# twke18/SPML

Measured on AMD Instinct MI355X. Metric: images/sec (513x513) + k-means iters/sec, higher is better.
Workload: dtype f32

## Files before the change

### include/spml_hip.h

```cpp
#ifndef SPML_HIP_H_
#define SPML_HIP_H_

#include <stddef.h>
#include <stdint.h>

#ifdef __cplusplus
extern "C" {
#endif

typedef enum spml_status {
  SPML_OK = 0,
  SPML_ERR_INVALID_ARG = -1,
  SPML_ERR_UNSUPPORTED = -2,
  SPML_ERR_WORKSPACE = -3,
  SPML_ERR_LAUNCH = -4
} spml_status;

const char* spml_status_string(int status);

#define SPML_ABI_VERSION 8
int spml_abi_version(void);

int spml_set_deterministic(int on);
int spml_get_deterministic(void);
// ... 224 lines not shown


int spml_hl8_from_f32(const float* x, int64_t rows, int C, float* bound,
                      int compute_bound, void* out, void* stream);

int spml_hl8_weight_transposed_f32(const float* w, int Cout, int taps, int Cin,
                                   const float* bound, void* out, void* stream);

int spml_conv_hl8_supported(int K, int N, int taps);

int spml_conv_hl8_f32(const void* a, const float* a_bound, const void* b,
                      const float* b_bound, const float* addend,
                      const unsigned char* addend_mask, float* out,
                      int n_img, int H, int W, int K, int N, int taps, int dilation,
                      void* stream);

int spml_conv_hl8_stats_layout(int n_img, int H, int W, int K, int N, int taps,
                               int* chunks, int* chunk_rows);
int spml_conv_hl8_stats_f32(const void* a, const float* a_bound, const void* b,
                            const float* b_bound, float* out, float* chunk_stats,
                            float* zero_me, int n_img, int H, int W, int K, int N,
                            int taps, int dilation, void* stream);

int spml_conv_wgrad_hl8_supported(int K, int N, int taps);
size_t spml_conv_wgrad_workspace_bytes(int n_img, int H, int W, int K, int N, int taps);
int spml_conv_wgrad_hl8_f32(const void* dy, const float* dy_bound, const void* x,
                            const float* x_bound, float* dw, int n_img, int H, int W,
                            int K, int N, int taps, int dilation, void* ws,
                            size_t ws_bytes, void* stream);

int spml_conv_wgrad_pyramid_hl8_supported(int K, int N, int branches);
int spml_conv_tap_gather_f32(const float* z, const float* bias, float* out, int n_img, int H,
                             int W, int N, int branches, const int* dilations, void* stream);
size_t spml_conv_wgrad_pyramid_workspace_bytes(int n_img, int H, int W, int K, int N,
                                               int branches);
int spml_conv_wgrad_pyramid_hl8_f32(const void* dy, const float* dy_bound, const void* x,
                                    const float* x_bound, float* dw, int n_img, int H, int W,
                                    int K, int N, int branches, const int* dilations,
                                    void* ws, size_t ws_bytes, void* stream);

int spml_bn_stats_ext_f32(const float* x, int64_t R, int C, float* mean, float* m2,
                          float* cmax, float* cmin, void* ws, size_t ws_bytes,
                          void* stream);

int spml_bn_stats_ext_chunks_f32(const float* chunk_stats, int chunks, int chunk_rows,
                                 int64_t R, int C, float* mean, float* m2, float* cmax,
// ... 30 lines not shown

int spml_bn_fwd_hl8_f32(const float* x, const float* residual, const float* residual_bound,
                        int64_t R, int C, const float* gamma, const float* beta,
                        float* running_mean, float* running_var, float momentum, float eps,
                        int relu, float* y, void* y_hl8, float* y_bound,
                        unsigned char* relu_mask, float* mean, float* invstd, float* cmax,
                        float* cmin, void* ws, size_t ws_bytes, void* stream);

int spml_bn_fwd_hl8_chunks_f32(const float* x, const float* chunk_stats, int chunks,
                               int chunk_rows, const float* residual,
                               const float* residual_bound, int64_t R, int C,
                               const float* gamma, const float* beta, float* running_mean,
                               float* running_var, float momentum, float eps, int relu,
                               float* y, void* y_hl8, float* y_bound,
                               unsigned char* relu_mask, float* mean, float* invstd,
                               float* cmax, float* cmin, void* stream);

int spml_bn_bwd_hl8_f32(const float* dy, const float* y, const unsigned char* relu_mask,
                        const float* x, int64_t R, int C, const float* mean,
                        const float* invstd, const float* gamma, const float* cmax,
                        const float* cmin, float* d_gamma, float* d_beta, float* dx,
                        void* dx_hl8, float* dx_bound, float* d_residual, void* ws,
                        size_t ws_bytes, void* stream);

int spml_conv_hl8_pyramid_f32(const void* a, const float* a_bound, const void* b,
                              const float* b_bound, const float* bias, const float* addend,
                              float* out,
                              int n_img, int H, int W, int K, int N, int groups,
                              const int* dilations, void* stream);
int spml_hl8_weight_transposed_into_f32(const float* w, int Cout, int taps, int Cin,
                                        const float* bound, void* out, int taps_total,
                                        int tap_offset, void* stream);
int spml_absmax_bound_f32(const float* x, int64_t n, float* bound, int zero_first,
                          void* stream);

int spml_hl8_weight_set_f32(const float* const* w, const int* cout, const int* cin,
                            const int* taps, int n, float* bounds, void* const* fwd,
                            void* const* transposed, void* stream);

int spml_bn_finalize_ranks_f32(const float* stats, int world, int C, float eps,
                               float momentum, float* running_mean, float* running_var,
                               float* mean, float* invstd, float* total_count, void* stream);

int spml_conv_hl8_affine_f32(const void* a, const float* a_bound, const void* b,
                             const float* b_bound, const float* bias, const float* addend,
                             int relu, float* out, float* out_bound, int n_img, int H,
// ... 76 lines not shown
```

### spml_amd/_ffi.py

```python
import ctypes
import os
import threading
from ctypes import c_char_p, c_double, c_float, c_int, c_int64, c_size_t, c_void_p

import torch

_HERE = os.path.dirname(os.path.abspath(__file__))
LIB_PATH = os.environ.get('SPML_HIP_LIB') or os.path.join(_HERE, 'lib', 'libspml_hip.so')

_lib = None
_lock = threading.Lock()

_P = c_void_p
_SIGNATURES = {
    'spml_status_string': (c_char_p, [c_int]),
    'spml_abi_version': (c_int, []),
    'spml_normalize_concat_loc_f32': (c_int, [_P, c_int, c_int, c_int, c_int, _P, _P, _P, _P, _P]),
    'spml_normalize_concat_loc_bwd_f32': (c_int, [_P, c_int, c_int, c_int, c_int, _P, _P, _P, _P, _P, _P]),
    'spml_normalize_concat_local_f32': (c_int, [_P, c_int, c_int, c_int, c_int, _P, c_int, _P, _P, _P, _P]),
    'spml_normalize_concat_local_nhwc_supported': (c_int, [c_int, c_int]),
    'spml_normalize_concat_local_nhwc_f32': (c_int, [_P, c_int, c_int, c_int, c_int, _P, c_int, _P, _P, _P, _P]),
    'spml_normalize_concat_local_nhwc_bwd_f32': (c_int, [_P, c_int, c_int, c_int, c_int, _P, c_int, _P, _P, _P,
                                                         _P, _P]),
    'spml_normalize_concat_local_bwd_f32': (c_int, [_P, c_int, c_int, c_int, c_int, _P, c_int, _P, _P, _P,
# ... 32 lines not shown
    'spml_segsort_nll_batched_workspace_bytes': (c_size_t, [c_int, _P, _P, c_int]),
    'spml_segsort_nll_batched_fwd_f32': (c_int, [_P, _P, _P, _P, _P, _P, _P, c_int, c_int, c_float, c_int,
                                                 _P, _P, _P, c_size_t, _P]),
    'spml_segsort_nll_batched_bwd_f32': (c_int, [_P, _P, _P, _P, _P, _P, _P, c_int, c_int, c_float, c_int,
                                                 _P, _P, _P, _P, _P, c_size_t, _P]),
    'spml_topk_workspace_bytes': (c_size_t, [c_int64, c_int64, c_int, c_int]),
    'spml_topk_affinity_f32': (c_int, [_P, c_int64, _P, c_int64, c_int, c_int, _P, _P, _P, c_float,
                                       _P, _P, _P, c_size_t, _P]),
    'spml_affinity_workspace_bytes': (c_size_t, [c_int, c_int, c_int64]),
    'spml_affinity_transition_f32': (c_int, [_P, c_int, c_int, c_int64, c_float, c_int, _P, _P, c_size_t,
                                             _P]),
    'spml_bn_workspace_bytes': (c_size_t, [c_int64, c_int]),
    'spml_bn_act_fwd_f32': (c_int, [_P, _P, c_int64, c_int, _P, _P, _P, _P, c_float, c_float, c_int, _P, _P, _P,
                                    _P, c_size_t, _P]),
    'spml_bn_act_bwd_f32': (c_int, [_P, _P, _P, c_int64, c_int, _P, _P, _P, _P, _P, _P, _P, _P, c_size_t, _P]),
    'spml_hl8_from_f32': (c_int, [_P, c_int64, c_int, _P, c_int, _P, _P]),
    'spml_hl8_weight_transposed_f32': (c_int, [_P, c_int, c_int, c_int, _P, _P, _P]),
    'spml_conv_hl8_supported': (c_int, [c_int, c_int, c_int]),
    'spml_conv_hl8_f32': (c_int, [_P, _P, _P, _P, _P, _P, _P, c_int, c_int, c_int, c_int, c_int, c_int, c_int, _P]),
    'spml_conv_hl8_stats_layout': (c_int, [c_int, c_int, c_int, c_int, c_int, c_int, _P, _P]),
    'spml_conv_hl8_stats_f32': (c_int, [_P, _P, _P, _P, _P, _P, _P, c_int, c_int, c_int, c_int, c_int, c_int, c_int, _P]),
    'spml_bn_fwd_hl8_chunks_f32': (c_int, [_P, _P, c_int, c_int, _P, _P, c_int64, c_int, _P, _P, _P, _P, c_float, c_float,
                                           c_int, _P, _P, _P, _P, _P, _P, _P, _P, _P]),
    'spml_conv_wgrad_hl8_supported': (c_int, [c_int, c_int, c_int]),
    'spml_conv_wgrad_workspace_bytes': (c_size_t, [c_int, c_int, c_int, c_int, c_int, c_int]),
    'spml_conv_wgrad_hl8_f32': (c_int, [_P, _P, _P, _P, _P, c_int, c_int, c_int, c_int, c_int, c_int, c_int, _P,
                                        c_size_t, _P]),
    'spml_conv_wgrad_pyramid_hl8_supported': (c_int, [c_int, c_int, c_int]),
    'spml_conv_tap_gather_f32': (c_int, [_P, _P, _P, c_int, c_int, c_int, c_int, c_int, _P, _P]),
    'spml_conv_wgrad_pyramid_workspace_bytes': (c_size_t, [c_int, c_int, c_int, c_int, c_int, c_int]),
    'spml_conv_wgrad_pyramid_hl8_f32': (c_int, [_P, _P, _P, _P, _P, c_int, c_int, c_int, c_int, c_int, c_int, _P, _P,
                                                c_size_t, _P]),
    'spml_bn_stats_ext_f32': (c_int, [_P, c_int64, c_int, _P, _P, _P, _P, _P, c_size_t, _P]),
    'spml_bn_stats_ext_chunks_f32': (c_int, [_P, c_int, c_int, c_int64, c_int, _P, _P, _P, _P, _P]),
    'spml_bn_finalize_f32': (c_int, [_P, _P, c_int, c_double, c_float, c_float, _P, _P, _P, _P]),
    'spml_bn_act_apply_hl8_f32': (c_int, [_P, _P, _P, c_int64, c_int, _P, _P, _P, _P, _P, _P, c_int, _P, _P, _P, _P,
                                          _P]),
    'spml_bn_act_bwd_reduce_ext_f32': (c_int, [_P, _P, _P, _P, c_int64, c_int, _P, _P, _P, _P, _P, _P, c_size_t, _P]),
    'spml_bn_act_bwd_apply_hl8_f32': (c_int, [_P, _P, _P, _P, c_int64, c_int, _P, _P, _P, _P, _P, _P, _P, _P,
                                              c_double, _P, _P, _P, _P, _P, _P]),
    'spml_bn_fwd_hl8_f32': (c_int, [_P, _P, _P, c_int64, c_int, _P, _P, _P, _P, c_float, c_float, c_int, _P, _P, _P, _P,
                                    _P, _P, _P, _P, _P, c_size_t, _P]),
    'spml_bn_bwd_hl8_f32': (c_int, [_P, _P, _P, _P, c_int64, c_int, _P, _P, _P, _P, _P, _P, _P, _P, _P, _P, _P, _P,
                                    c_size_t, _P]),
    'spml_conv_hl8_pyramid_f32': (c_int, [_P, _P, _P, _P, _P, _P, _P, c_int, c_int, c_int, c_int, c_int, c_int, _P,
                                          _P]),
# ... 849 lines not shown
  def __init__(self, data, chunks, chunk_rows, bound):
    self.data, self.chunks, self.chunk_rows, self.bound = data, chunks, chunk_rows, bound


def conv_hl8_stats(a, b, n_img, h, w, taps, dilation=1):
  import ctypes
  k, n = a.channels, b.rows
  chunks, rows = ctypes.c_int(0), ctypes.c_int(0)
  if os.environ.get('SPML_CONV_BN_STATS') == '0' or lib().spml_conv_hl8_stats_layout(
      n_img, h, w, k, n, taps, ctypes.byref(chunks), ctypes.byref(rows)) != 0:
    return conv_hl8(a, b, n_img, h, w, taps, dilation), None
  if a.rows != n_img * h * w or b.channels != taps * k:
    raise SpmlHipError('conv_hl8_stats: operand shapes do not match')
  dev = a.data.device
  out = torch.empty((n_img, n, h, w), dtype=torch.float32, device=dev, memory_format=torch.channels_last)
  st = torch.empty((4, chunks.value, n), dtype=torch.float32, device=dev)
  bound = _f32(1, dev)
  check(lib().spml_conv_hl8_stats_f32(ptr(a.data), c_void_p(a.bound.data_ptr()), ptr(b.data),
                                      c_void_p(b.bound.data_ptr()), _ptr_any(out), _dp(st), _dp(bound), n_img, h, w,
                                      k, n, taps, dilation, stream_ptr()), 'spml_conv_hl8_stats_f32')
  return out, ChunkStats(st, chunks.value, rows.value, bound)


def conv_wgrad_hl8_supported(k, n, taps):
  return bool(lib().spml_conv_wgrad_hl8_supported(int(k), int(n), int(taps)))


_wgrad_ws = {}


def conv_wgrad_hl8(dy, x, n_img, h, w, taps, dilation=1):
  n, k = dy.channels, x.channels
  if dy.rows != n_img * h * w or x.rows != dy.rows:
    raise SpmlHipError('conv_wgrad_hl8: operand shapes do not match')
  need = lib().spml_conv_wgrad_workspace_bytes(n_img, h, w, k, n, taps)
  key = (dy.data.device.index, torch.cuda.current_stream().cuda_stream)
  ws = _wgrad_ws.get(key)
  if ws is None or ws.numel() < need:
    ws = workspace(need, dy.data.device)
    _wgrad_ws[key] = ws
  side = 3 if taps == 9 else 1
  dw = torch.empty((n, k, side, side), dtype=torch.float32, device=dy.data.device,
                   memory_format=torch.channels_last)
  check(lib().spml_conv_wgrad_hl8_f32(ptr(dy.data), c_void_p(dy.bound.data_ptr()), ptr(x.data),
                                      c_void_p(x.bound.data_ptr()), _ptr_any(dw), n_img, h, w, k, n, taps,
                                      dilation, ptr(ws), ws.numel(), stream_ptr()), 'spml_conv_wgrad_hl8_f32')
# ... 65 lines not shown


def bn_finalize(mean, m2, count, eps, momentum, running_mean, running_var):
  invstd = torch.empty_like(mean)
  check(lib().spml_bn_finalize_f32(_dp(mean), _dp(m2), mean.numel(), float(count), float(eps), float(momentum),
                                   _dp(running_mean), _dp(running_var), _dp(invstd), stream_ptr()),
        'spml_bn_finalize_f32')
  return invstd


def bn_act_apply_hl8(x, rows, channels, residual, residual_bound, mean, invstd, gamma, beta, cmax, cmin, relu,
                     want_f32, want_hl8, like=None, want_mask=False):
  y = torch.empty_like(x if like is None else like) if want_f32 else None
  yh = torch.empty((rows * channels * 4,), dtype=torch.uint8, device=x.device) if want_hl8 else None
  bound = _f32(1, x.device)
  mask = torch.empty((rows * (channels // 4),), dtype=torch.uint8, device=x.device) if want_mask else None
  check(lib().spml_bn_act_apply_hl8_f32(
      _ptr_any(x), _ptr_any(residual, True), _dp(residual_bound), rows, channels, _dp(mean), _dp(invstd),
      ptr(gamma, torch.float32), ptr(beta, torch.float32), _dp(cmax), _dp(cmin), int(bool(relu)), _ptr_any(y, True),
      _dp(yh), _dp(bound), _dp(mask), stream_ptr()), 'spml_bn_act_apply_hl8_f32')
  return y, (Hl8(yh, bound, rows, channels) if want_hl8 else None), bound, mask


def bn_act_bwd_reduce_ext(dy, y, relu_mask, x, rows, channels, mean, invstd):
  st = torch.empty((3, channels), dtype=torch.float32, device=dy.device)
  ws = _bn_workspace(rows, channels, dy.device)
  check(lib().spml_bn_act_bwd_reduce_ext_f32(
      _ptr_any(dy), _ptr_any(y, True), _dp(relu_mask), _ptr_any(x), rows, channels,
      _dp(mean), _dp(invstd), _dp(st[0]), _dp(st[1]), _dp(st[2]), ptr(ws), ws.numel(), stream_ptr()),
        'spml_bn_act_bwd_reduce_ext_f32')
  return st


def bn_act_bwd_apply_hl8(dy, y, relu_mask, x, rows, channels, mean, invstd, gamma, s0, s1, max_dz, cmax, cmin, count,
                         want_dx_f32=False, want_dx_hl8=True, want_dres=False):
  dx = torch.empty_like(dy) if want_dx_f32 else None
  dxh = torch.empty((rows * channels * 4,), dtype=torch.uint8, device=dy.device) if want_dx_hl8 else None
  bound = _f32(1, dy.device) if want_dx_hl8 else None
  dres = torch.empty_like(dy) if want_dres else None
  count, count_dev = _count_args(count)
  check(lib().spml_bn_act_bwd_apply_hl8_f32(
      _ptr_any(dy), _ptr_any(y, True), _dp(relu_mask), _ptr_any(x), rows, channels,
      _dp(mean), _dp(invstd), ptr(gamma, torch.float32), _dp(s0), _dp(s1), _dp(max_dz), _dp(cmax), _dp(cmin),
      count, count_dev, _ptr_any(dx, True), _dp(dxh), _dp(bound), _ptr_any(dres, True), stream_ptr()),
        'spml_bn_act_bwd_apply_hl8_f32')
  return dx, (Hl8(dxh, bound, rows, channels) if want_dx_hl8 else None), dres


def bn_fwd_hl8(x, rows, channels, residual, residual_bound, gamma, beta, running_mean, running_var, momentum, eps,
               relu, want_f32, want_hl8, want_mask, chunk_stats=None):
  y = torch.empty_like(x) if want_f32 else None
  yh = torch.empty((rows * channels * 4,), dtype=torch.uint8, device=x.device) if want_hl8 else None
  bound = _f32(1, x.device) if chunk_stats is None else chunk_stats.bound
  mask = torch.empty((rows * (channels // 4),), dtype=torch.uint8, device=x.device) if want_mask else None
  st = torch.empty((4, channels), dtype=torch.float32, device=x.device)
  if chunk_stats is not None:
    check(lib().spml_bn_fwd_hl8_chunks_f32(
        _ptr_any(x), _dp(chunk_stats.data), chunk_stats.chunks, chunk_stats.chunk_rows, _ptr_any(residual, True),
        _dp(residual_bound), rows, channels, ptr(gamma, torch.float32), ptr(beta, torch.float32), _dp(running_mean),
        _dp(running_var), float(momentum), float(eps), int(bool(relu)), _ptr_any(y, True), _dp(yh), _dp(bound),
        _dp(mask), _dp(st[0]), _dp(st[1]), _dp(st[2]), _dp(st[3]), stream_ptr()), 'spml_bn_fwd_hl8_chunks_f32')
    return y, (Hl8(yh, bound, rows, channels) if want_hl8 else None), bound, mask, (st[0], st[1], st[2], st[3])
  ws = _bn_workspace(rows, channels, x.device)
  check(lib().spml_bn_fwd_hl8_f32(
      _ptr_any(x), _ptr_any(residual, True), _dp(residual_bound), rows, channels, ptr(gamma, torch.float32),
      ptr(beta, torch.float32), _dp(running_mean), _dp(running_var), float(momentum), float(eps), int(bool(relu)),
      _ptr_any(y, True), _dp(yh), _dp(bound), _dp(mask), _dp(st[0]), _dp(st[1]), _dp(st[2]), _dp(st[3]), ptr(ws),
      ws.numel(), stream_ptr()), 'spml_bn_fwd_hl8_f32')
  return y, (Hl8(yh, bound, rows, channels) if want_hl8 else None), bound, mask, (st[0], st[1], st[2], st[3])


def bn_bwd_hl8(dy, relu_mask, x, rows, channels, saved, gamma, want_dres=False):
  mean, invstd, cmax, cmin = saved
  dxh = torch.empty((rows * channels * 4,), dtype=torch.uint8, device=dy.device)
  bound = _f32(1, dy.device)
  dres = torch.empty_like(dy) if want_dres else None
  dgb = torch.empty((2, channels), dtype=torch.float32, device=dy.device)
  ws = _bn_workspace(rows, channels, dy.device)
  check(lib().spml_bn_bwd_hl8_f32(
      _ptr_any(dy), c_void_p(0), _dp(relu_mask), _ptr_any(x), rows, channels, _dp(mean), _dp(invstd),
      ptr(gamma, torch.float32), _dp(cmax), _dp(cmin), _dp(dgb[0]), _dp(dgb[1]), c_void_p(0), _dp(dxh), _dp(bound),
      _ptr_any(dres, True), ptr(ws), ws.numel(), stream_ptr()), 'spml_bn_bwd_hl8_f32')
  return Hl8(dxh, bound, rows, channels), dres, dgb[0], dgb[1]


def conv_hl8_pyramid_dgrad(dy, weights, dilations, n_img, h, w):
  groups = len(weights)
  cout, cin = weights[0].shape[0], weights[0].shape[1]
  dev = dy.data.device
  bound = torch.empty((1,), dtype=torch.float32, device=dev)
  wl = [wt.detach().contiguous(memory_format=torch.channels_last) for wt in weights]
  for g, wt in enumerate(wl):
    check(lib().spml_absmax_bound_f32(_ptr_any(wt), wt.numel(), _dp(bound), int(g == 0), stream_ptr()),
          'spml_absmax_bound_f32')
  b = torch.empty((cin * 9 * groups * cout * 4,), dtype=torch.uint8, device=dev)
  for g, wt in enumerate(wl):
    check(lib().spml_hl8_weight_transposed_into_f32(_ptr_any(wt), cout, 9, cin, _dp(bound), ptr(b), 9 * groups, 9 * g,
                                                    stream_ptr()), 'spml_hl8_weight_transposed_into_f32')
  out = torch.empty((n_img, cin, h, w), dtype=torch.float32, device=dev, memory_format=torch.channels_last)
# ... 161 lines not shown
```

### spml_amd/csrc/bn_act.hip

```cpp
#include "common.hpp"

namespace spml {
namespace {


__device__ __forceinline__ float4v relu_mask_bits(float4v dz, const unsigned char* __restrict__ mask, size_t row,
                                                  int C, int q) {
  const unsigned m = mask[row * (size_t)(C >> 2) + q];
#pragma unroll
  for (int e = 0; e < 4; ++e) dz[e] = (m >> e) & 1u ? dz[e] : 0.f;
  return dz;
}

__device__ __forceinline__ float bn_pow2_scale(float bound) {
  if (!(bound > 0.f) || bound > 1e38f) return 1.f;
  int e;
  (void)frexpf(bound, &e);
  e = 14 - e;
  e = e < -100 ? -100 : (e > 100 ? 100 : e);
  return ldexpf(1.f, e);
}

__device__ __forceinline__ void store_hl8_quad(uint2* __restrict__ out, size_t row, int C, int q, float4v v,
                                               float s) {
// ... 790 lines not shown
    return SPML_ERR_UNSUPPORTED;
  if (!ws || ws_bytes < spml_bn_workspace_bytes(R, C)) return SPML_ERR_WORKSPACE;
  const int chunks = bn_chunks(R, C), cq = bn_cq(C), crows = bn_chunk_rows(R, C), arows = bn_apply_rows(R, C);
  float* pa = static_cast<float*>(ws);
  float* pb = pa + (size_t)chunks * C;
  float* pc = pb + (size_t)chunks * C;
  float* max_dz = pc + (size_t)chunks * C;
  hipStream_t s = (hipStream_t)stream;
  const int mask = y ? 1 : (relu_mask ? 2 : 0);
  SPML_BN_PARTIAL1(mask, dim3(((C >> 2) + cq - 1) / cq, chunks), dim3(256), 0, s, x, dy, y, mean, R, C, cq, crows, pa, pb,
                   relu_mask, pc, (float*)nullptr, dx_hl8 ? dx_bound : (float*)nullptr);
  hipLaunchKernelGGL(bn_merge<1>, dim3((C + kMergeCh - 1) / kMergeCh), dim3(kMergeCh * kMergeLanes), 0, s, pa, pb, R,
                     C, chunks, crows, invstd, d_beta, d_gamma, BnFinal{0, 0.f, 0.f, nullptr, nullptr},
                     (const float*)pc, (const float*)nullptr, max_dz, (float*)nullptr,
                     BnBound{dx_hl8 ? dx_bound : nullptr, nullptr, gamma, nullptr, mean, cmax, cmin, (float)(1.0 / (double)R)});
  if (!dx && !dx_hl8 && !d_residual) return launch_status();
  const dim3 grid(((C >> 2) + cq - 1) / cq, (unsigned)((R + arows - 1) / arows));
  SPML_BN_BY_MASK(bn_bwd_apply, mask, grid, dim3(256), 0, s, dy, y, x, R, C, cq, arows, mean, invstd, gamma,
                  (const float*)d_beta, (const float*)d_gamma, (float)(1.0 / (double)R), (const float*)nullptr, dx,
                  d_residual, relu_mask, static_cast<uint2*>(dx_hl8), (const float*)dx_bound);
  return launch_status();
}

extern "C" int spml_bn_finalize_ranks_f32(const float* stats, int world, int C, float eps, float momentum,
                                          float* running_mean, float* running_var, float* mean, float* invstd,
                                          float* total_count, void* stream) {
  if (!stats || !mean || !invstd || world < 1 || C <= 0) return SPML_ERR_INVALID_ARG;
  hipLaunchKernelGGL(bn_finalize_ranks, dim3((C + 255) / 256), dim3(256), 0, (hipStream_t)stream, C, world, stats, eps,
                     momentum, running_mean, running_var, mean, invstd, total_count);
  return launch_status();
}
```

### spml_amd/csrc/conv.hip

```cpp
#include "common.hpp"

#include <math.h>
#include <stdlib.h>

#ifndef SPML_CONV_EXP
#define SPML_CONV_EXP 0
#endif

namespace spml {
namespace {

typedef const __attribute__((address_space(1))) void* gptr_t;
typedef __attribute__((address_space(3))) void* lptr_t;

__device__ uint4 g_zero_page[16];

__device__ __forceinline__ float pow2_scale(float bound) {
  if (!(bound > 0.f) || bound > 1e38f) return 1.f;
  int e;
  (void)frexpf(bound, &e);
  e = 14 - e;
  e = e < -100 ? -100 : (e > 100 ? 100 : e);
  return ldexpf(1.f, e);
}

__device__ __forceinline__ void split_unscaled(const float (&v)[8], float s, half8& h, half8& l) {
#pragma unroll
  for (int j = 0; j < 8; ++j) {
    const float x = v[j] * s;
    const _Float16 hj = (_Float16)x;
    h[j] = hj;
    l[j] = (_Float16)(x - (float)hj);
  }
// ... 111 lines not shown
      th[(2 * tu + 1) * 8 + (co & 7)] = ll.e[e];
    }
  }
}

struct ConvArgs {
  const uint4* a;
  const uint4* b;
  const float* a_bound;
  const float* b_bound;
  const float* addend;
  const unsigned char* addend_mask;
  const float* bias;
  int relu;
  float* out_bound;
  float* out;
  int64_t R;
  int H, W, K, N, taps, dil;
  int n_col_tiles, n_tiles;
  int dils[4];
  int tap_groups;
  float* stats;
  float* stats_zero;
};

template <int RB, int kStages, int WGS, int RG, bool CHUNK = false, int NC = 4>
__global__ __launch_bounds__(64 * NC * RG, WGS) void conv_gemm(const ConvArgs a) {
  constexpr int kABlocks = 2 * RB * RG;
  constexpr int kBlocks = kABlocks + 4 * NC;
  constexpr int kStage = kBlocks * 1024;
  constexpr int kWaves = NC * RG;
  constexpr int NQ = (kABlocks + kWaves - 1) / kWaves;
  extern __shared__ __attribute__((aligned(1024))) unsigned char lds[];
  const int lane = threadIdx.x & 63, wave = threadIdx.x >> 6;
  const int wc = wave % NC, wg = wave / NC;
  const int lr = lane & 31;
  const int drow = lane >> 2, dpiece = ((lane & 3) - (drow >> 2)) & 3;
  const unsigned foff_h = (unsigned)((lr >> 4) * 1024 + 16 * (4 * (lr & 15) + (((lane >> 5) * 2 + ((lr & 15) >> 2)) & 3)));
  const unsigned foff_l = (unsigned)((lr >> 4) * 1024 + 16 * (4 * (lr & 15) + (((lane >> 5) * 2 + 1 + ((lr & 15) >> 2)) & 3)));

  unsigned long long exp_c0 = 0, exp_r0 = 0;
  if (SPML_CONV_EXP & 16) { exp_c0 = __builtin_amdgcn_s_memtime(); exp_r0 = __builtin_amdgcn_s_memrealtime(); }
  int t = blockIdx.x;
  if ((a.n_tiles & 7) == 0) t = (t & 7) * (a.n_tiles >> 3) + (t >> 3);
  const int row_tile = t / a.n_col_tiles, col_tile = t - row_tile * a.n_col_tiles;
  const int64_t m0 = (int64_t)row_tile * (RG * RB * 32);
  const int n0 = col_tile * (64 * NC) + wc * 64;
  const int k8 = a.K >> 3, nk = a.K >> 4;
  const int hw = a.H * a.W;
  const int tpg = a.taps / (int)gridDim.y, tap_begin = (int)blockIdx.y * tpg, tap_end = tap_begin + tpg;
// ... 142 lines not shown
      acc[i][1] = mfma32(ah[c], bh1, acc[i][1]);
      } else {
        asm volatile("" :: "v"(al[c]), "v"(ah[c]), "v"(bh0), "v"(bl0), "v"(bh1), "v"(bl1));
      }
    }
    if (CHUNK && (s & 63) == 63) {
#pragma unroll
      for (int i = 0; i < RB; ++i)
#pragma unroll
        for (int j = 0; j < 2; ++j)
#pragma unroll
          for (int r = 0; r < 16; ++r) { tot[i][j][r] += acc[i][j][r]; acc[i][j][r] = 0.f; }
    }
  }
  if (CHUNK) {
#pragma unroll
    for (int i = 0; i < RB; ++i)
#pragma unroll
      for (int j = 0; j < 2; ++j)
#pragma unroll
        for (int r = 0; r < 16; ++r) acc[i][j][r] += tot[i][j][r];
  }

  const float mult = 1.0f / ((a.a_bound ? pow2_scale(*a.a_bound) : 1.f) * (a.b_bound ? pow2_scale(*a.b_bound) : 1.f));
  float vmax = 0.f;
#pragma unroll
  for (int i = 0; i < RB; ++i)
#pragma unroll
    for (int r = 0; r < 16; ++r) {
      const int64_t row = m0 + (wg * RB + i) * 32 + acc_row(r, lane);
      if (row < a.R) {
#pragma unroll
        for (int j = 0; j < 2; ++j) {
          const size_t o = (size_t)row * a.N + n0 + j * 32 + lr;
          float v = acc[i][j][r] * mult;
          if (gridDim.y > 1) {
            if (a.bias && blockIdx.y == 0) v += a.bias[n0 + j * 32 + lr];
            unsafeAtomicAdd(a.out + o, v);
            continue;
          }
          if (a.bias) v += a.bias[n0 + j * 32 + lr];
          if (a.addend) {
            float ad = a.addend[o];
            if (a.addend_mask) ad = (a.addend_mask[o >> 2] >> (o & 3)) & 1 ? ad : 0.f;
            v += ad;
          }
// ... 41 lines not shown
          dst[0] = mean;
          dst[plane] = m2;
          dst[2 * plane] = hi;
          dst[3 * plane] = lo;
        }
      }
    }
  }
  if ((SPML_CONV_EXP & 32) && blockIdx.x == 7 && lane == 0) {
#pragma unroll
    for (int i = 0; i < 4; ++i) a.out[8 + wave * 4 + i] = (float)exp_ph[i];
  }
  if ((SPML_CONV_EXP & 16) && blockIdx.x == 7 && threadIdx.x == 0) {
    a.out[0] = (float)(__builtin_amdgcn_s_memtime() - exp_c0);
    a.out[1] = (float)(__builtin_amdgcn_s_memrealtime() - exp_r0);
  }
  if (a.out_bound) {
#pragma unroll
    for (int o = 32; o > 0; o >>= 1) vmax = fmaxf(vmax, __shfl_xor(vmax, o, kWave));
    if (lane == 0) atomicMax(reinterpret_cast<unsigned*>(a.out_bound), __float_as_uint(vmax));
  }
}

template <int RB, int kStages, int WGS, int RG = 1, bool CHUNK = false, int NC = 4>
int launch_conv(const ConvArgs& a0, hipStream_t s) {
  ConvArgs a = a0;
  a.n_col_tiles = a.N / (64 * NC);
  const int64_t row_tiles = (a.R + RG * RB * 32 - 1) / (RG * RB * 32);
  a.n_tiles = (int)(row_tiles * a.n_col_tiles);
  auto kern = conv_gemm<RB, kStages, WGS, RG, CHUNK, NC>;
  const int lds = kStages * (2 * RB * RG + 4 * NC) * 1024;
  (void)hipFuncSetAttribute(reinterpret_cast<const void*>(kern), hipFuncAttributeMaxDynamicSharedMemorySize, lds);
  const int groups = a.tap_groups > 1 ? a.tap_groups : 1;
  if (groups > 1 && hipMemsetAsync(a.out, 0, (size_t)a.R * a.N * sizeof(float), s) != hipSuccess) return SPML_ERR_LAUNCH;
  hipLaunchKernelGGL(kern, dim3(a.n_tiles, groups), dim3(64 * NC * RG), lds, s, a);
  return launch_status();
}

template <bool CHUNK>
int launch_conv_narrow(const ConvArgs& c, hipStream_t s) {
  if ((c.N & 127) == 0) return launch_conv<CHUNK ? 3 : 4, 3, 2, 2, CHUNK, 2>(c, s);
  const char* e = getenv("SPML_CONV_NARROW_RB");
  if (e && e[0] == '3') return launch_conv<3, 3, 1, 4, CHUNK, 1>(c, s);
  return launch_conv<2, 3, 2, 4, CHUNK, 1>(c, s);
}

inline bool chunk_long_reduction(int64_t k_total) {
  int64_t min_k = 4096;
  if (const char* e = getenv("SPML_CONV_CHUNK_MIN_K")) min_k = atoll(e);
  return k_total >= min_k;
}

inline int pick_rb(int64_t R, int N) {
// ... 392 lines not shown
                                       float* out, float* chunk_stats, float* zero_me, int n_img, int H, int W,
                                       int K, int N, int taps, int dilation, void* stream) {
  if (!a || !b || !out || !chunk_stats || n_img <= 0 || H <= 0 || W <= 0 || dilation < 1) return SPML_ERR_INVALID_ARG;
  int chunks = 0, rows = 0;
  if (spml_conv_hl8_stats_layout(n_img, H, W, K, N, taps, &chunks, &rows) != SPML_OK || !al16(a) || !al16(b) ||
      !al16(out))
    return SPML_ERR_UNSUPPORTED;
  ConvArgs c{};
  c.a = static_cast<const uint4*>(a);
  c.b = static_cast<const uint4*>(b);
  c.a_bound = a_bound;
  c.b_bound = b_bound;
  c.out = out;
  c.stats = chunk_stats;
  c.stats_zero = zero_me;
  c.R = (int64_t)n_img * H * W;
  c.H = H; c.W = W; c.K = K; c.N = N; c.taps = taps; c.dil = dilation;
  hipStream_t s = (hipStream_t)stream;
  if (chunk_long_reduction((int64_t)c.K * c.taps)) return launch_conv<3, 3, 2, 1, true>(c, s);
  switch (rows / 32) {
    case 3: return launch_conv<3, 3, 2>(c, s);
    case 5: return launch_conv<5, 3, 2>(c, s);
    default: return launch_conv<4, 3, 2>(c, s);
  }
}

extern "C" int spml_conv_hl8_affine_f32(const void* a, const float* a_bound, const void* b, const float* b_bound,
                                        const float* bias, const float* addend, int relu, float* out,
                                        float* out_bound, int n_img, int H, int W, int K, int N, int taps,
                                        int dilation, void* stream) {
  if (!a || !b || !out || n_img <= 0 || H <= 0 || W <= 0 || dilation < 1) return SPML_ERR_INVALID_ARG;
  if (!spml_conv_hl8_supported(K, N, taps) || !al16(a) || !al16(b) || !al16(out) || (addend && !al16(addend)))
    return SPML_ERR_UNSUPPORTED;
  ConvArgs c{};
  c.a = static_cast<const uint4*>(a);
  c.b = static_cast<const uint4*>(b);
  c.a_bound = a_bound;
  c.b_bound = b_bound;
  c.bias = bias;
  c.addend = addend;
  c.relu = relu;
  c.out = out;
  c.out_bound = out_bound;
  c.R = (int64_t)n_img * H * W;
  c.H = H; c.W = W; c.K = K; c.N = N; c.taps = taps; c.dil = dilation;
  hipStream_t s = (hipStream_t)stream;
// ... 216 lines not shown
```

### spml_amd/mc_bottleneck.py

```python
import os

import torch
import torch.distributed as dist

from spml_amd import _ffi
from spml_amd._cache import BoundedCache


def _group_of(bn):
  if isinstance(bn, torch.nn.SyncBatchNorm) and dist.is_available() and dist.is_initialized():
    return bn.process_group if bn.process_group is not None else dist.group.WORLD
  return None


def available(block, x, allow_forward_only=True):
  if os.environ.get('SPML_NO_MC_CONV') == '1' or not (x.is_cuda and x.dtype == torch.float32 and x.dim() == 4):
    return False
  if not block.training or block.stride != 1 or not x.is_contiguous(memory_format=torch.channels_last):
    return False
  convs = [block.conv1, block.conv2, block.conv3] + ([block.downsample[0]] if block.downsample is not None else [])
  if os.environ.get('SPML_MC_NARROW_UNITS') == '0' and any(
      (c.in_channels & 255) or (c.out_channels & 255) for c in convs):
    return False
  bns = [block.bn1, block.bn2, block.bn3] + ([block.downsample[1]] if block.downsample is not None else [])
# ... 93 lines not shown
      return
    if gathered is None:
      st = _ffi.bn_stats_ext(a, rows, channels, chunk_stats=chunk_stats)
      allst = torch.empty((world * 3, channels), dtype=st.dtype, device=st.device)
      dist.all_gather_into_tensor(allst, st[:3], group=group)
      allst = allst.view(world, 3, channels)
    else:
      allst, st = gathered
    if bn.num_batches_tracked is not None:
      if counters is not None:
        counters.append(bn.num_batches_tracked)
      else:
        bn.num_batches_tracked.add_(1)
    mean, invstd, self.count = _ffi.bn_finalize_ranks(allst, bn.eps, bn.momentum, bn.running_mean, bn.running_var)
    _touch(bn)
    cmax, cmin = st[3], st[4]
    self.y, self.yh, self.bound, self.mask = _ffi.bn_act_apply_hl8(
        a, rows, channels, residual, residual_bound, mean, invstd, bn.weight, bn.bias, cmax, cmin, relu,
        want_f32, want_hl8, want_mask=relu)
    self.saved = (mean, invstd, cmax, cmin)


def _bn_backward(dy, a, rows, channels, gamma, saved, count, group, world, mask, want_dres=False,
                 want_dx_f32=False):
  if world == 1:
    dxh, dres, d_gamma, d_beta = _ffi.bn_bwd_hl8(dy, mask, a, rows, channels, saved, gamma, want_dres=want_dres)
    return None, dxh, dres, d_gamma, d_beta
  mean, invstd, cmax, cmin = saved
  st = _ffi.bn_act_bwd_reduce_ext(dy, None, mask, a, rows, channels, mean, invstd)
  local = st[:2].clone()
  d_beta, d_gamma = local[0], local[1]
  dist.all_reduce(st[:2], group=group)
  dx, dxh, dres = _ffi.bn_act_bwd_apply_hl8(dy, None, mask, a, rows, channels, mean, invstd, gamma, st[0], st[1],
                                            st[2], cmax, cmin, count, want_dx_f32=want_dx_f32, want_dx_hl8=True,
                                            want_dres=want_dres)
  return dx, dxh, dres, d_gamma, d_beta


def sync_pair(bn_a, a_a, chunk_a, bn_b, a_b, chunk_b, rows, channels):
  group = _group_of(bn_a)
  if group is None or _group_of(bn_b) is not group or dist.get_world_size(group) == 1:
    return None, None
  world = dist.get_world_size(group)
  st_a = _ffi.bn_stats_ext(a_a, rows, channels, chunk_stats=chunk_a)
  st_b = _ffi.bn_stats_ext(a_b, rows, channels, chunk_stats=chunk_b)
  loc = torch.cat([st_a[:3], st_b[:3]], dim=1)
  allst = torch.empty((world * 3, 2 * channels), dtype=loc.dtype, device=loc.device)
  dist.all_gather_into_tensor(allst, loc, group=group)
  allst = allst.view(world, 3, 2 * channels)
  return (allst[:, :, :channels].contiguous(), st_a), (allst[:, :, channels:].contiguous(), st_b)


# ... 90 lines not shown
    rows = n * h * w
    (xh_d, xh_b, a1, y1_d, y1_b, a2, y2_d, y2_b, a3, m3, m1, m2, w1t_d, w1t_b, w2t_d, w2t_b, w3t_d, w3t_b, g1, g2,
     g3) = t[:21]
    s1, s2, s3 = t[21:25], t[25:29], t[29:33]
    has_ds = len(t) > 33
    H = _ffi.Hl8
    xh, y1h, y2h = H(xh_d, xh_b, rows, cin), H(y1_d, y1_b, rows, width), H(y2_d, y2_b, rows, width)
    w1t, w2t, w3t = H(w1t_d, w1t_b, cin, width), H(w2t_d, w2t_b, width, 9 * width), H(w3t_d, w3t_b, width, cout)
    if not d_out.is_contiguous(memory_format=torch.channels_last):
      d_out = d_out.contiguous(memory_format=torch.channels_last)
    need_x = ctx.needs_input_grad[1]
    m = ctx.bn_meta
    dwd = dgd = dbd = dad = None
    pair = has_ds and m[2][2] > 1 and m[3][1] is m[2][1]
    if pair:
      da3, dad, dg3, db3, dgd, dbd = _bn_backward_pair(d_out, m3, a3, g3, s3, t[33], t[36], t[37:41], rows, cout,
                                                       m[2][0], m[2][1])
      dres = None
    else:
      _, da3, dres, dg3, db3 = _bn_backward(d_out, a3, rows, cout, g3, s3, m[2][0], m[2][1], m[2][2], m3,
                                            want_dres=has_ds)
    side = _side_stream(d_out.device)
    dw3 = _wgrad(side, da3, y2h, n, h, w, 1)
    dy2 = _ffi.conv_hl8(da3, w3t, n, h, w, 1)
    del da3
    _, da2, _, dg2, db2 = _bn_backward(dy2, a2, rows, width, g2, s2, m[1][0], m[1][1], m[1][2], m2)
    dw2 = _wgrad(side, da2, y1h, n, h, w, 9, dil)
    dy1 = _ffi.conv_hl8(da2, w2t, n, h, w, 9, dil)
    del da2, dy2
    _, da1, _, dg1, db1 = _bn_backward(dy1, a1, rows, width, g1, s1, m[0][0], m[0][1], m[0][2], m1)
    dw1 = _wgrad(side, da1, xh, n, h, w, 1)
    dx = None
    if has_ds:
      ad, wdt_d, wdt_b, gd = t[33:37]
      sd = t[37:41]
      if not pair:
        _, dad, _, dgd, dbd = _bn_backward(dres, ad, rows, cout, gd, sd, m[3][0], m[3][1], m[3][2], None)
      dwd = _wgrad(side, dad, xh, n, h, w, 1)
      if need_x:
        dx = _ffi.conv_hl8(da1, w1t, n, h, w, 1)
        dx = _ffi.conv_hl8(dad, H(wdt_d, wdt_b, cin, cout), n, h, w, 1, addend=dx)
    elif need_x:
      dx = _ffi.conv_hl8(da1, w1t, n, h, w, 1, addend=d_out, addend_mask=m3)
    if side is not None:
      torch.cuda.current_stream().wait_stream(side)
    return (None, dx, None, None, dw1, dg1, db1, dw2, dg2, db2, dw3, dg3, db3, dwd, dgd, dbd)


class _ConvBnAct(torch.autograd.Function):

  @staticmethod
  def forward(ctx, conv, bn, x, weight, gamma, beta):
    n, cin, h, w = x.shape
# ... 61 lines not shown
```

Before: 136.3.

## Fuse BN-backward reduction statistics into dgrad conv epilogue in bottleneck backward

Adds a BSTAT variant of the conv GEMM epilogue that, while storing the conv output, loads the BN input and ReLU mask and accumulates per-chunk sum(dz), sum(dz*(x-mean)) and max|dz|. BN backward then merges these chunk stats instead of making a separate reduction pass over dy and x. This is meant to remove one full read of the activation gradient and the saved input per BN layer in the bottleneck backward. In exchange the conv epilogue does extra loads, which raises register pressure and can lower conv occupancy.

```diff
diff --git a/include/spml_hip.h b/include/spml_hip.h
--- a/include/spml_hip.h
+++ b/include/spml_hip.h
@@ -270,6 +270,14 @@
                             float* zero_me, int n_img, int H, int W, int K, int N,
                             int taps, int dilation, void* stream);
 
+int spml_conv_hl8_bwd_stats_layout(int n_img, int H, int W, int K, int N, int taps,
+                                   int* chunks, int* chunk_rows);
+int spml_conv_hl8_bwd_stats_f32(const void* a, const float* a_bound, const void* b,
+                                const float* b_bound, float* out, const float* bn_x,
+                                const unsigned char* relu_mask, const float* bn_mean,
+                                float* chunk_stats, float* zero_me, int n_img, int H, int W,
+                                int K, int N, int taps, int dilation, void* stream);
+
 int spml_conv_wgrad_hl8_supported(int K, int N, int taps);
 size_t spml_conv_wgrad_workspace_bytes(int n_img, int H, int W, int K, int N, int taps);
 int spml_conv_wgrad_hl8_f32(const void* dy, const float* dy_bound, const void* x,
@@ -346,6 +354,17 @@
                         const float* cmin, float* d_gamma, float* d_beta, float* dx,
                         void* dx_hl8, float* dx_bound, float* d_residual, void* ws,
                         size_t ws_bytes, void* stream);
+
+int spml_bn_bwd_hl8_chunks_f32(const float* dy, const unsigned char* relu_mask, const float* x,
+                               const float* chunk_stats, int chunks, int chunk_rows, int64_t R,
+                               int C, const float* mean, const float* invstd, const float* gamma,
+                               const float* cmax, const float* cmin, float* d_gamma,
+                               float* d_beta, float* max_dz, float* dx, void* dx_hl8,
+                               float* dx_bound, float* d_residual, void* stream);
+
+int spml_bn_act_bwd_reduce_ext_chunks_f32(const float* chunk_stats, int chunks, int chunk_rows,
+                                          int64_t R, int C, const float* invstd, float* sum_dz,
+                                          float* sum_dz_xhat, float* max_dz, void* stream);
 
 int spml_conv_hl8_pyramid_f32(const void* a, const float* a_bound, const void* b,
                               const float* b_bound, const float* bias, const float* addend,
diff --git a/spml_amd/_ffi.py b/spml_amd/_ffi.py
--- a/spml_amd/_ffi.py
+++ b/spml_amd/_ffi.py
@@ -78,6 +78,12 @@
     'spml_conv_hl8_stats_f32': (c_int, [_P, _P, _P, _P, _P, _P, _P, c_int, c_int, c_int, c_int, c_int, c_int, c_int, _P]),
     'spml_bn_fwd_hl8_chunks_f32': (c_int, [_P, _P, c_int, c_int, _P, _P, c_int64, c_int, _P, _P, _P, _P, c_float, c_float,
                                            c_int, _P, _P, _P, _P, _P, _P, _P, _P, _P]),
+    'spml_conv_hl8_bwd_stats_layout': (c_int, [c_int, c_int, c_int, c_int, c_int, c_int, _P, _P]),
+    'spml_conv_hl8_bwd_stats_f32': (c_int, [_P, _P, _P, _P, _P, _P, _P, _P, _P, _P, c_int, c_int, c_int, c_int, c_int,
+                                            c_int, c_int, _P]),
+    'spml_bn_bwd_hl8_chunks_f32': (c_int, [_P, _P, _P, _P, c_int, c_int, c_int64, c_int, _P, _P, _P, _P, _P, _P, _P, _P,
+                                           _P, _P, _P, _P, _P]),
+    'spml_bn_act_bwd_reduce_ext_chunks_f32': (c_int, [_P, c_int, c_int, c_int64, c_int, _P, _P, _P, _P, _P]),
     'spml_conv_wgrad_hl8_supported': (c_int, [c_int, c_int, c_int]),
     'spml_conv_wgrad_workspace_bytes': (c_size_t, [c_int, c_int, c_int, c_int, c_int, c_int]),
     'spml_conv_wgrad_hl8_f32': (c_int, [_P, _P, _P, _P, _P, c_int, c_int, c_int, c_int, c_int, c_int, c_int, _P,
@@ -973,6 +979,27 @@
   return out, ChunkStats(st, chunks.value, rows.value, bound)
 
 
+def conv_hl8_bwd_stats(a, b, n_img, h, w, taps, dilation, bn_x, relu_mask, bn_mean):
+  import ctypes
+  k, n = a.channels, b.rows
+  chunks, rows = ctypes.c_int(0), ctypes.c_int(0)
+  if relu_mask is None or os.environ.get('SPML_CONV_BN_BWD_STATS') == '0' or lib().spml_conv_hl8_bwd_stats_layout(
+      n_img, h, w, k, n, taps, ctypes.byref(chunks), ctypes.byref(rows)) != 0:
+    return conv_hl8(a, b, n_img, h, w, taps, dilation), None
+  if a.rows != n_img * h * w or b.channels != taps * k or bn_x.numel() != a.rows * n or \
+      relu_mask.numel() != a.rows * (n // 4) or bn_mean.numel() != n:
+    raise SpmlHipError('conv_hl8_bwd_stats: operand shapes do not match')
+  dev = a.data.device
+  out = torch.empty((n_img, n, h, w), dtype=torch.float32, device=dev, memory_format=torch.channels_last)
+  st = torch.empty((3, chunks.value, n), dtype=torch.float32, device=dev)
+  bound = _f32(1, dev)
+  check(lib().spml_conv_hl8_bwd_stats_f32(ptr(a.data), c_void_p(a.bound.data_ptr()), ptr(b.data),
+                                          c_void_p(b.bound.data_ptr()), _ptr_any(out), _ptr_any(bn_x), _dp(relu_mask),
+                                          _dp(bn_mean), _dp(st), _dp(bound), n_img, h, w, k, n, taps, dilation,
+                                          stream_ptr()), 'spml_conv_hl8_bwd_stats_f32')
+  return out, ChunkStats(st, chunks.value, rows.value, bound)
+
+
 def conv_wgrad_hl8_supported(k, n, taps):
   return bool(lib().spml_conv_wgrad_hl8_supported(int(k), int(n), int(taps)))
 
@@ -1084,8 +1111,13 @@
   return y, (Hl8(yh, bound, rows, channels) if want_hl8 else None), bound, mask
 
 
-def bn_act_bwd_reduce_ext(dy, y, relu_mask, x, rows, channels, mean, invstd):
+def bn_act_bwd_reduce_ext(dy, y, relu_mask, x, rows, channels, mean, invstd, chunk_stats=None):
   st = torch.empty((3, channels), dtype=torch.float32, device=dy.device)
+  if chunk_stats is not None:
+    check(lib().spml_bn_act_bwd_reduce_ext_chunks_f32(
+        _dp(chunk_stats.data), chunk_stats.chunks, chunk_stats.chunk_rows, rows, channels, _dp(invstd), _dp(st[0]),
+        _dp(st[1]), _dp(st[2]), stream_ptr()), 'spml_bn_act_bwd_reduce_ext_chunks_f32')
+    return st
   ws = _bn_workspace(rows, channels, dy.device)
   check(lib().spml_bn_act_bwd_reduce_ext_f32(
       _ptr_any(dy), _ptr_any(y, True), _dp(relu_mask), _ptr_any(x), rows, channels,
@@ -1132,11 +1164,20 @@
   return y, (Hl8(yh, bound, rows, channels) if want_hl8 else None), bound, mask, (st[0], st[1], st[2], st[3])
 
 
-def bn_bwd_hl8(dy, relu_mask, x, rows, channels, saved, gamma, want_dres=False):
+def bn_bwd_hl8(dy, relu_mask, x, rows, channels, saved, gamma, want_dres=False, chunk_stats=None):
   mean, invstd, cmax, cmin = saved
   dxh = torch.empty((rows * channels * 4,), dtype=torch.uint8, device=dy.device)
+  dres = torch.empty_like(dy) if want_dres else None
+  if chunk_stats is not None:
+    bound = chunk_stats.bound
+    dgb = torch.empty((3, channels), dtype=torch.float32, device=dy.device)
+    check(lib().spml_bn_bwd_hl8_chunks_f32(
+        _ptr_any(dy), _dp(relu_mask), _ptr_any(x), _dp(chunk_stats.data), chunk_stats.chunks, chunk_stats.chunk_rows,
+        rows, channels, _dp(mean), _dp(invstd), ptr(gamma, torch.float32), _dp(cmax), _dp(cmin), _dp(dgb[0]),
+        _dp(dgb[1]), _dp(dgb[2]), c_void_p(0), _dp(dxh), _dp(bound), _ptr_any(dres, True), stream_ptr()),
+          'spml_bn_bwd_hl8_chunks_f32')
+    return Hl8(dxh, bound, rows, channels), dres, dgb[0], dgb[1]
   bound = _f32(1, dy.device)
-  dres = torch.empty_like(dy) if want_dres else None
   dgb = torch.empty((2, channels), dtype=torch.float32, device=dy.device)
   ws = _bn_workspace(rows, channels, dy.device)
   check(lib().spml_bn_bwd_hl8_f32(
diff --git a/spml_amd/csrc/bn_act.hip b/spml_amd/csrc/bn_act.hip
--- a/spml_amd/csrc/bn_act.hip
+++ b/spml_amd/csrc/bn_act.hip
@@ -836,6 +836,53 @@
   return launch_status();
 }
 
+extern "C" int spml_bn_bwd_hl8_chunks_f32(const float* dy, const unsigned char* relu_mask, const float* x,
+                                          const float* chunk_stats, int chunks, int chunk_rows, int64_t R, int C,
+                                          const float* mean, const float* invstd, const float* gamma,
+                                          const float* cmax, const float* cmin, float* d_gamma, float* d_beta,
+                                          float* max_dz, float* dx, void* dx_hl8, float* dx_bound, float* d_residual,
+                                          void* stream) {
+  if (!dy || !x || !chunk_stats || !mean || !invstd || !gamma || !cmax || !cmin || !d_gamma || !d_beta || !max_dz ||
+      R <= 0 || C <= 0 || chunks <= 0 || chunk_rows <= 0 || (int64_t)chunks * chunk_rows < R ||
+      (int64_t)(chunks - 1) * chunk_rows >= R || (dx_hl8 && !dx_bound))
+    return SPML_ERR_INVALID_ARG;
+  if ((C & 7) || !bn_ok(dy) || !bn_ok(x) || (dx && !bn_ok(dx)) || (dx_hl8 && !bn_ok(dx_hl8)) ||
+      (d_residual && !bn_ok(d_residual)) || !bn_ok(mean))
+    return SPML_ERR_UNSUPPORTED;
+  const int cq = bn_cq(C), arows = bn_apply_rows(R, C);
+  const float* pa = chunk_stats;
+  const float* pb = pa + (size_t)chunks * C;
+  const float* pc = pb + (size_t)chunks * C;
+  hipStream_t s = (hipStream_t)stream;
+  const int mask = relu_mask ? 2 : 0;
+  hipLaunchKernelGGL(bn_merge<1>, dim3((C + kMergeCh - 1) / kMergeCh), dim3(kMergeCh * kMergeLanes), 0, s, pa, pb, R,
+                     C, chunks, chunk_rows, invstd, d_beta, d_gamma, BnFinal{0, 0.f, 0.f, nullptr, nullptr}, pc,
+                     (const float*)nullptr, max_dz, (float*)nullptr,
+                     BnBound{dx_hl8 ? dx_bound : nullptr, nullptr, gamma, nullptr, mean, cmax, cmin, (float)(1.0 / (double)R)});
+  if (!dx && !dx_hl8 && !d_residual) return launch_status();
+  const dim3 grid(((C >> 2) + cq - 1) / cq, (unsigned)((R + arows - 1) / arows));
+  SPML_BN_BY_MASK(bn_bwd_apply, mask, grid, dim3(256), 0, s, dy, (const float*)nullptr, x, R, C, cq, arows, mean, invstd,
+                  gamma, (const float*)d_beta, (const float*)d_gamma, (float)(1.0 / (double)R), (const float*)nullptr, dx,
+                  d_residual, relu_mask, static_cast<uint2*>(dx_hl8), (const float*)dx_bound);
+  return launch_status();
+}
+
+extern "C" int spml_bn_act_bwd_reduce_ext_chunks_f32(const float* chunk_stats, int chunks, int chunk_rows, int64_t R,
+                                                     int C, const float* invstd, float* sum_dz, float* sum_dz_xhat,
+                                                     float* max_dz, void* stream) {
+  if (!chunk_stats || !invstd || !sum_dz || !sum_dz_xhat || !max_dz || R <= 0 || C <= 0 || chunks <= 0 ||
+      chunk_rows <= 0 || (int64_t)chunks * chunk_rows < R || (int64_t)(chunks - 1) * chunk_rows >= R)
+    return SPML_ERR_INVALID_ARG;
+  const float* pa = chunk_stats;
+  const float* pb = pa + (size_t)chunks * C;
+  const float* pc = pb + (size_t)chunks * C;
+  hipLaunchKernelGGL(bn_merge<1>, dim3((C + kMergeCh - 1) / kMergeCh), dim3(kMergeCh * kMergeLanes), 0,
+                     (hipStream_t)stream, pa, pb, R, C, chunks, chunk_rows, invstd, sum_dz, sum_dz_xhat,
+                     BnFinal{0, 0.f, 0.f, nullptr, nullptr}, pc, (const float*)nullptr, max_dz, (float*)nullptr,
+                     BnBound{});
+  return launch_status();
+}
+
 extern "C" int spml_bn_finalize_ranks_f32(const float* stats, int world, int C, float eps, float momentum,
                                           float* running_mean, float* running_var, float* mean, float* invstd,
                                           float* total_count, void* stream) {
diff --git a/spml_amd/csrc/conv.hip b/spml_amd/csrc/conv.hip
--- a/spml_amd/csrc/conv.hip
+++ b/spml_amd/csrc/conv.hip
@@ -9,6 +9,8 @@
 
 namespace spml {
 namespace {
+
+constexpr int BSTAT_BATCH = 8;
 
 typedef const __attribute__((address_space(1))) void* gptr_t;
 typedef __attribute__((address_space(3))) void* lptr_t;
@@ -166,10 +168,15 @@
   int tap_groups;
   float* stats;
   float* stats_zero;
+  const float* bstat_x;
+  const unsigned char* bstat_mask;
+  const float* bstat_mean;
+  float* bstats;
 };
 
-template <int RB, int kStages, int WGS, int RG, bool CHUNK = false, int NC = 4>
+template <int RB, int kStages, int WGS, int RG, bool CHUNK = false, int NC = 4, bool BSTAT = false>
 __global__ __launch_bounds__(64 * NC * RG, WGS) void conv_gemm(const ConvArgs a) {
+  static_assert(!BSTAT || (RG == 1 && NC == 4), "backward statistics: a wave owns its 64 columns over the whole tile");
   constexpr int kABlocks = 2 * RB * RG;
   constexpr int kBlocks = kABlocks + 4 * NC;
   constexpr int kStage = kBlocks * 1024;
@@ -358,6 +365,83 @@
         for (int r = 0; r < 16; ++r) acc[i][j][r] += tot[i][j][r];
   }
 
+  if constexpr (BSTAT) {
+    constexpr int kB = BSTAT_BATCH, kBatches = RB * 16 / kB;
+    const unsigned N = (unsigned)a.N;
+    const unsigned rows_here = (unsigned)(m0 + RB * 32 < a.R ? (int64_t)RB * 32 : a.R - m0);
+    const unsigned tile_bytes = rows_here * N * 4u;
+    const size_t t0e = (size_t)m0 * N;
+    const auto rx = __builtin_amdgcn_make_buffer_rsrc(const_cast<float*>(a.bstat_x + t0e), 0, (int)tile_bytes, 0x00020000);
+    const auto rm = __builtin_amdgcn_make_buffer_rsrc(const_cast<unsigned char*>(a.bstat_mask + (t0e >> 2)), 0,
+                                                      (int)(tile_bytes >> 4), 0x00020000);
+    const auto ro = __builtin_amdgcn_make_buffer_rsrc(a.out + t0e, 0, (int)tile_bytes, 0x00020000);
+    unsigned tid = threadIdx.x;
+    asm volatile("" : "+v"(tid));
+    const unsigned up = (tid >> 5) & 1u;
+    const unsigned col = (unsigned)(col_tile * (64 * NC)) + ((tid >> 6) * 64u + (tid & 31u));
+    const unsigned lo = (up * 4u * N + col) * 4u;
+    const unsigned lm = up * N + (col >> 2);
+    const unsigned bit = 1u << (tid & 3u);
+    float xv[2][kB][2];
+    unsigned mv[2][kB][2];
+    auto fetch = [&](int b, float (&x)[kB][2], unsigned (&m)[kB][2]) {
+#pragma unroll
+      for (int e = 0; e < kB; ++e) {
+        const int idx = b * kB + e;
+        const unsigned ro_e = (unsigned)((idx >> 4) * 32 + acc_row(idx & 15, 0)) * N;
+        const unsigned vo = lo + ro_e * 4u, vm = lm + (ro_e >> 2);
+        x[e][0] = __builtin_bit_cast(float, __builtin_amdgcn_raw_buffer_load_b32(rx, vo, 0, 0));
+        x[e][1] = __builtin_bit_cast(float, __builtin_amdgcn_raw_buffer_load_b32(rx, vo + 128u, 0, 0));
+        m[e][0] = __builtin_amdgcn_raw_buffer_load_b8(rm, vm, 0, 0);
+        m[e][1] = __builtin_amdgcn_raw_buffer_load_b8(rm, vm + 8u, 0, 0);
+      }
+    };
+    fetch(0, xv[0], mv[0]);
+    __builtin_amdgcn_sched_barrier(0);
+    if (a.stats_zero && blockIdx.x == 0 && threadIdx.x == 0) *a.stats_zero = 0.f;
+    const float mu[2] = {a.bstat_mean[col], a.bstat_mean[col + 32]};
+    const float mult = 1.0f / ((a.a_bound ? pow2_scale(*a.a_bound) : 1.f) * (a.b_bound ? pow2_scale(*a.b_bound) : 1.f));
+    float s0[2] = {0.f, 0.f}, s1[2] = {0.f, 0.f}, mx[2] = {0.f, 0.f};
+#pragma unroll
+    for (int b = 0; b < kBatches; ++b) {
+      if (b + 1 < kBatches) fetch(b + 1, xv[(b + 1) & 1], mv[(b + 1) & 1]);
+      __builtin_amdgcn_sched_barrier(0);
+      float t0[2] = {0.f, 0.f}, t1[2] = {0.f, 0.f};
+#pragma unroll
+      for (int e = 0; e < kB; ++e) {
+        const int idx = b * kB + e, i = idx >> 4, r = idx & 15;
+        const unsigned vo = lo + (unsigned)(i * 32 + acc_row(r, 0)) * N * 4u;
+#pragma unroll
+        for (int j = 0; j < 2; ++j) {
+          const float v = acc[i][j][r] * mult;
+          __builtin_amdgcn_raw_buffer_store_b32(__builtin_bit_cast(unsigned, v), ro, vo + 128u * j, 0, 0);
+          const float dz = (mv[b & 1][e][j] & bit) ? v : 0.f;
+          t0[j] += dz;
+          t1[j] += dz * (xv[b & 1][e][j] - mu[j]);
+          mx[j] = fmaxf(mx[j], fabsf(dz));
+        }
+      }
+#pragma unroll
+      for (int j = 0; j < 2; ++j) { s0[j] += t0[j]; s1[j] += t1[j]; }
+      asm volatile("" : "+v"(s0[0]), "+v"(s0[1]), "+v"(s1[0]), "+v"(s1[1]), "+v"(mx[0]), "+v"(mx[1]));
+      __builtin_amdgcn_sched_barrier(0);
+    }
+    const size_t plane = (size_t)gridDim.x / a.n_col_tiles * a.N;
+#pragma unroll
+    for (int j = 0; j < 2; ++j) {
+      const float p0 = s0[j] + __shfl_xor(s0[j], 32, kWave);
+      const float p1 = s1[j] + __shfl_xor(s1[j], 32, kWave);
+      const float pm = fmaxf(mx[j], __shfl_xor(mx[j], 32, kWave));
+      if (!up) {
+        float* dst = a.bstats + (size_t)row_tile * a.N + col + j * 32;
+        dst[0] = p0;
+        dst[plane] = p1;
+        dst[2 * plane] = pm;
+      }
+    }
+    return;
+  }
+
   const float mult = 1.0f / ((a.a_bound ? pow2_scale(*a.a_bound) : 1.f) * (a.b_bound ? pow2_scale(*a.b_bound) : 1.f));
   float vmax = 0.f;
 #pragma unroll
@@ -445,13 +529,13 @@
   }
 }
 
-template <int RB, int kStages, int WGS, int RG = 1, bool CHUNK = false, int NC = 4>
+template <int RB, int kStages, int WGS, int RG = 1, bool CHUNK = false, int NC = 4, bool BSTAT = false>
 int launch_conv(const ConvArgs& a0, hipStream_t s) {
   ConvArgs a = a0;
   a.n_col_tiles = a.N / (64 * NC);
   const int64_t row_tiles = (a.R + RG * RB * 32 - 1) / (RG * RB * 32);
   a.n_tiles = (int)(row_tiles * a.n_col_tiles);
-  auto kern = conv_gemm<RB, kStages, WGS, RG, CHUNK, NC>;
+  auto kern = conv_gemm<RB, kStages, WGS, RG, CHUNK, NC, BSTAT>;
   const int lds = kStages * (2 * RB * RG + 4 * NC) * 1024;
   (void)hipFuncSetAttribute(reinterpret_cast<const void*>(kern), hipFuncAttributeMaxDynamicSharedMemorySize, lds);
   const int groups = a.tap_groups > 1 ? a.tap_groups : 1;
@@ -890,6 +974,44 @@
     case 3: return launch_conv<3, 3, 2>(c, s);
     case 5: return launch_conv<5, 3, 2>(c, s);
     default: return launch_conv<4, 3, 2>(c, s);
+  }
+}
+
+extern "C" int spml_conv_hl8_bwd_stats_layout(int n_img, int H, int W, int K, int N, int taps, int* chunks,
+                                              int* chunk_rows) {
+  return spml_conv_hl8_stats_layout(n_img, H, W, K, N, taps, chunks, chunk_rows);
+}
+
+extern "C" int spml_conv_hl8_bwd_stats_f32(const void* a, const float* a_bound, const void* b, const float* b_bound,
+                                           float* out, const float* bn_x, const unsigned char* relu_mask,
+                                           const float* bn_mean, float* chunk_stats, float* zero_me, int n_img, int H,
+                                           int W, int K, int N, int taps, int dilation, void* stream) {
+  if (!a || !b || !out || !bn_x || !relu_mask || !bn_mean || !chunk_stats || n_img <= 0 || H <= 0 || W <= 0 ||
+      dilation < 1)
+    return SPML_ERR_INVALID_ARG;
+  int chunks = 0, rows = 0;
+  if (spml_conv_hl8_bwd_stats_layout(n_img, H, W, K, N, taps, &chunks, &rows) != SPML_OK || !al16(a) || !al16(b) ||
+      !al16(out) || !al16(bn_x))
+    return SPML_ERR_UNSUPPORTED;
+  ConvArgs c{};
+  c.a = static_cast<const uint4*>(a);
+  c.b = static_cast<const uint4*>(b);
+  c.a_bound = a_bound;
+  c.b_bound = b_bound;
+  c.out = out;
+  c.bstat_x = bn_x;
+  c.bstat_mask = relu_mask;
+  c.bstat_mean = bn_mean;
+  c.bstats = chunk_stats;
+  c.stats_zero = zero_me;
+  c.R = (int64_t)n_img * H * W;
+  c.H = H; c.W = W; c.K = K; c.N = N; c.taps = taps; c.dil = dilation;
+  hipStream_t s = (hipStream_t)stream;
+  if (chunk_long_reduction((int64_t)c.K * c.taps)) return launch_conv<3, 3, 2, 1, true, 4, true>(c, s);
+  switch (rows / 32) {
+    case 3: return launch_conv<3, 3, 2, 1, false, 4, true>(c, s);
+    case 5: return launch_conv<5, 3, 2, 1, false, 4, true>(c, s);
+    default: return launch_conv<4, 3, 2, 1, false, 4, true>(c, s);
   }
 }
 
diff --git a/spml_amd/mc_bottleneck.py b/spml_amd/mc_bottleneck.py
--- a/spml_amd/mc_bottleneck.py
+++ b/spml_amd/mc_bottleneck.py
@@ -139,12 +139,14 @@
 
 
 def _bn_backward(dy, a, rows, channels, gamma, saved, count, group, world, mask, want_dres=False,
-                 want_dx_f32=False):
+                 want_dx_f32=False, chunk_stats=None):
   if world == 1:
-    dxh, dres, d_gamma, d_beta = _ffi.bn_bwd_hl8(dy, mask, a, rows, channels, saved, gamma, want_dres=want_dres)
+    dxh, dres, d_gamma, d_beta = _ffi.bn_bwd_hl8(dy, mask, a, rows, channels, saved, gamma, want_dres=want_dres,
+                                                 chunk_stats=chunk_stats)
     return None, dxh, dres, d_gamma, d_beta
   mean, invstd, cmax, cmin = saved
-  st = _ffi.bn_act_bwd_reduce_ext(dy, None, mask, a, rows, channels, mean, invstd)
+  st = _ffi.bn_act_bwd_reduce_ext(dy, None, mask, a, rows, channels, mean, invstd,
+                                  chunk_stats=chunk_stats)
   local = st[:2].clone()
   d_beta, d_gamma = local[0], local[1]
   dist.all_reduce(st[:2], group=group)
@@ -281,13 +283,13 @@
                                             want_dres=has_ds)
     side = _side_stream(d_out.device)
     dw3 = _wgrad(side, da3, y2h, n, h, w, 1)
-    dy2 = _ffi.conv_hl8(da3, w3t, n, h, w, 1)
+    dy2, c2 = _ffi.conv_hl8_bwd_stats(da3, w3t, n, h, w, 1, 1, a2, m2, s2[0])
     del da3
-    _, da2, _, dg2, db2 = _bn_backward(dy2, a2, rows, width, g2, s2, m[1][0], m[1][1], m[1][2], m2)
+    _, da2, _, dg2, db2 = _bn_backward(dy2, a2, rows, width, g2, s2, m[1][0], m[1][1], m[1][2], m2, chunk_stats=c2)
     dw2 = _wgrad(side, da2, y1h, n, h, w, 9, dil)
-    dy1 = _ffi.conv_hl8(da2, w2t, n, h, w, 9, dil)
+    dy1, c1 = _ffi.conv_hl8_bwd_stats(da2, w2t, n, h, w, 9, dil, a1, m1, s1[0])
     del da2, dy2
-    _, da1, _, dg1, db1 = _bn_backward(dy1, a1, rows, width, g1, s1, m[0][0], m[0][1], m[0][2], m1)
+    _, da1, _, dg1, db1 = _bn_backward(dy1, a1, rows, width, g1, s1, m[0][0], m[0][1], m[0][2], m1, chunk_stats=c1)
     dw1 = _wgrad(side, da1, xh, n, h, w, 1)
     dx = None
     if has_ds:
```

New measurement: 137.7, median of 6. 1.0% higher.
